# LeCAR-Lab/dial-mpc

Measured on NVIDIA H100. Metric: sample-steps/s (Nsample*Hsample/wall-s) per MPC reverse_once, Go2, higher is better.
Workload: dtype f32

## Files before the change

### dial_mpc_b200/csrc/dial_device.cuh

```cuda
#pragma once

#include <stdint.h>
#include <math.h>
#include "../../include/dial_b200.h"

#ifdef DIAL_HOST_EMUL
#include "warp_emul.h"
#define DEV inline
#define HD inline
inline float __fmaf_rn(float a, float b, float c) { return a * b + c; }
inline float __fadd_rn(float a, float b) { return a + b; }
inline float __fmul_rn(float a, float b) { return a * b; }
inline float __fdiv_rn(float a, float b) { return a / b; }
inline float __fsub_rn(float a, float b) { return a - b; }
inline double __dadd_rn(double a, double b) { return a + b; }
inline double __dsub_rn(double a, double b) { return a - b; }
inline double __dmul_rn(double a, double b) { return a * b; }
inline double __ddiv_rn(double a, double b) { return a / b; }
#else
#define HD __host__ __device__ __forceinline__
#define DEV __device__ __forceinline__
DEV void syncwarp() { __syncwarp(); }
DEV float shfl(float v, int src) { return __shfl_sync(0xffffffffu, v, src); }
DEV float shfl_xor(float v, int m) { return __shfl_xor_sync(0xffffffffu, v, m); }
// ... 8 lines not shown
extern "C" void emul_trace(int kind, int val);
#define DIAL_TRACE(lane, kind, val) do { if ((lane) == 0) emul_trace(kind, val); } while (0)
#else
#define DIAL_TRACE(lane, kind, val) do { } while (0)
#endif

#define DIAL_MAXCHAIN 12
#define DIAL_MAXLEVEL 28
#define DIAL_MAXE 32
#define DIAL_MINVAL 1e-15f
#define DIAL_MINIMP 1e-4f
#define DIAL_MAXIMP 0.9999f

enum { JNT_FREE = 0, JNT_BALL = 1, JNT_SLIDE = 2, JNT_HINGE = 3 };
enum { PAIR_PLANE_SPHERE = 0, PAIR_PLANE_CAPSULE = 1, PAIR_SPHERE_SPHERE = 2, PAIR_SPHERE_CAPSULE = 3, PAIR_CAPSULE_CAPSULE = 4 };

struct alignas(16) DevModel {
  dial_model_desc m;
  int32_t maxdepth;
  int32_t nroot, root_body[4];
  float root_invmass[4];
  int32_t body_rootidx[DIAL_MAXB];
  int32_t body_ndesc[DIAL_MAXB];
  int32_t dof_level[DIAL_MAXV], nlevel;
  int32_t level_adr[DIAL_MAXLEVEL + 1], level_dofs[DIAL_MAXV];
  uint32_t dof_ancmask[DIAL_MAXV];
  uint32_t body_dofmask[DIAL_MAXB];
  int32_t dof_actuator[DIAL_MAXV];
  int32_t dof_limited[DIAL_MAXV];
  int32_t con_pair[DIAL_MAXC], con_sub[DIAL_MAXC];
// ... 7 lines not shown
  int32_t star_nroot, star_nchain, star_maxlen;
  int32_t star_root[8], star_len[4], star_leaf[4], star_att[4];
  int32_t nedge;
  int32_t s_on, s_nrp, s_cs, s_rs, s_npos;
  int32_t s_pos[DIAL_MAXV];
  int32_t s_chain[DIAL_MAXV];
  int32_t s_depth[DIAL_MAXV];
  int32_t s_top[4];
  int32_t s_con_chain[DIAL_MAXC];
  int32_t o_Ms, o_Hs, o_Js, o_xs;
  int32_t sb_on, sb_nroot, sb_root[4], sb_top[4], sb_len[4], sb_att[4];
  int32_t o_xpos, o_xquat, o_xmat, o_xipos, o_cinert, o_cdof, o_cdofdot, o_cvel, o_cacc,
      o_cfrc, o_Mb, o_L, o_J, o_qpos, o_qvel, o_warm, o_ctrl, o_vec, o_frow, o_cpos,
      o_cframe, o_cdist, o_rcom, o_xch, o_crb, o_cfs, o_Md, o_Ld, o_Jd, o_Gd, o_frow2, o_cact, o_hcs, warp_floats;
  int32_t pad_[1];
};

struct alignas(16) DevPlan {
  dial_plan_desc c;
  int32_t pad_[3];
};

#define DIAL_TASK_AT(f) (offsetof(dial_plan_desc, f) - offsetof(dial_plan_desc, vel_cmd) == offsetof(dial_task, f))
static_assert(DIAL_TASK_AT(vel_cmd) && DIAL_TASK_AT(ang_cmd) && DIAL_TASK_AT(pos_tar) && DIAL_TASK_AT(gait_duty) &&
              DIAL_TASK_AT(gait_cadence) && DIAL_TASK_AT(gait_amplitude) && DIAL_TASK_AT(gait_phase) &&
              DIAL_TASK_AT(cmd_step) && DIAL_TASK_AT(cmd_vel) && DIAL_TASK_AT(cmd_ang) && DIAL_TASK_AT(n_stage) &&
              DIAL_TASK_AT(jump_dt) && DIAL_TASK_AT(pose_seq) && DIAL_TASK_AT(yaw_seq) &&
              DIAL_TASK_AT(contact_targets) && DIAL_TASK_AT(contact_radius) && DIAL_TASK_AT(n_user) &&
              DIAL_TASK_AT(user) &&
              offsetof(dial_plan_desc, user) + sizeof(float) * DIAL_MAXUSER - offsetof(dial_plan_desc, vel_cmd) == sizeof(dial_task),
// ... 437 lines not shown
    p = 1.00167406f + p * w; p = 2.83297682f + p * w;
  }
  return p * x;
}
DEV float jax_normal_legacy(uint32_t k0, uint32_t k1, uint32_t i, uint32_t n) {
  uint32_t bits = jax_bits_legacy(k0, k1, i, n);
  float f = __uint_as_float((bits >> 9) | 0x3F800000u) - 1.0f;
  const float lo = -0.99999994f;
  float u = fmaxf(lo, f * 2.0f + lo);
  return 1.41421356237f * erfinv_f32(u);
}

struct WarpCtx {
  const DevModel* M;
  const DevPlan* P;
  float* s;
  int lane;
  int nch;
  int ndesc;
  int mylevel;
  int parent;
  int midsync;
  int itersync;
  float* dbg;
  int chain[DIAL_MAXCHAIN];
  int s_pos;
  int s_col;
  int s_cb;
  int s_chain;
  int s_depth;
// ... 271 lines not shown
  syncwarp();
  float y = 0.f;
  if (w.nch > 0) {
    for (int c = 0; c < M.m.ncon; ++c) {
      const int kc = M.con_lastdof[c];
      if ((M.dof_ancmask[kc] >> lane) & 1u) {
        const int off = M.dof_nchain[kc] - w.nch;
#pragma unroll
        for (int e = 0; e < 4; ++e) y += Jc[(4 * c + e) * MC + off] * frow[4 * c + e];
      }
    }
  }
  return y;
}

DEV void kbi(float timestep, const float* solref, const float* solimp, float pos,
             float& k, float& b, float& imp) {
  float timeconst = fmaxf(solref[0], 2.f * timestep), dampratio = solref[1];
  float dmin = fminf(fmaxf(solimp[0], DIAL_MINIMP), DIAL_MAXIMP);
  float dmax = fminf(fmaxf(solimp[1], DIAL_MINIMP), DIAL_MAXIMP);
  float width = fmaxf(DIAL_MINVAL, solimp[2]);
  float mid = fminf(fmaxf(solimp[3], DIAL_MINIMP), DIAL_MAXIMP);
  float power = fmaxf(1.f, solimp[4]);
  k = 1.f / (dmax * dmax * timeconst * timeconst * dampratio * dampratio);
  b = 2.f / (dmax * timeconst);
  if (solref[0] <= 0.f) k = -solref[0] / (dmax * dmax);
  if (solref[1] <= 0.f) b = -solref[1] / dmax;
  float x = fabsf(pos) / width;
  float y;
  if (power == 2.f) {
    y = x < mid ? x * x / mid : 1.f - (1.f - x) * (1.f - x) / (1.f - mid);
  } else {
    float a_ = (1.f / powf(mid, power - 1.f)) * powf(x, power);
    float b_ = 1.f - (1.f / powf(1.f - mid, power - 1.f)) * powf(fmaxf(1.f - x, 0.f), power);
    y = x < mid ? a_ : b_;
  }
  imp = dmin + y * (dmax - dmin);
  imp = fminf(fmaxf(imp, dmin), dmax);
  if (x > 1.f) imp = dmax;
}

struct Solver {
  float qacc, Ma, grad, search, qfs, qas;
  float l_sign, l_D, l_aref, l_Jaref;
  float e_D, e_aref, e_Jaref;
  float gauss, cost, prev_cost, gradnorm2;
  float qfc;
};

DEV void update_constraint(WarpCtx& w, Solver& S) {
  float fl = (S.l_Jaref < 0.f) ? -S.l_D * S.l_Jaref : 0.f;
  float fe = (S.e_Jaref < 0.f) ? -S.e_D * S.e_Jaref : 0.f;
  float qfc = mul_JT(w, fe) + S.l_sign * fl;
  S.grad = S.Ma - S.qfs - qfc;
// ... 1090 lines not shown
}
DEV V3 frame_tangent(V3 n) {
  V3 alt = (n.y > -0.5f && n.y < 0.5f) ? v3(0, 1, 0) : v3(0, 0, 1);
  float bn;
  return vnormalize(alt - n * dot(n, alt), bn);
}

template <class SH = ShapeRT>
DEV void collide(WarpCtx& w) {
  const DevModel& M = *w.M;
  const dial_model_desc& m = M.m;
  const int lane = w.lane;
  if (lane >= SH::ncon(M)) return;
  const float* xpos = SM(xpos);
  const float* xmat = SM(xmat);
  const int k = M.con_pair[lane];
  const int g1 = m.pair_geom1[k], g2 = m.pair_geom2[k];
  const int b1 = m.geom_bodyid[g1], b2 = m.geom_bodyid[g2];
  const float* X1 = xmat + 9 * b1;
  const float* X2 = xmat + 9 * b2;
  const V3 gp1 = mat_apply(X1, m.geom_pos[g1]) + ld3(xpos + 3 * b1);
  const V3 gp2 = mat_apply(X2, m.geom_pos[g2]) + ld3(xpos + 3 * b2);
  const int kind = SH::pair_kind(M, k);
  V3 n, t1, p;
  float dist;
  if (kind == PAIR_PLANE_SPHERE || kind == PAIR_PLANE_CAPSULE) {
    n = mat_z(X1, m.geom_quat[g1]);
    const float radius = m.geom_size[g2][0];
    V3 center = gp2;
    if (kind == PAIR_PLANE_CAPSULE) {
      V3 ax = mat_z(X2, m.geom_quat[g2]);
      float bn;
      V3 bd = vnormalize(ax - n * dot(n, ax), bn);
// ... 34 lines not shown

template <int NL, int NR, class SH = ShapeRT>
DEV void physics_step(WarpCtx& w, bool integrate) {
  constexpr int MCU = (NL == 3 && NR == 6) ? 9 : DIAL_MAXCHAIN;
  const DevModel& M = *w.M;
  const dial_model_desc& m = M.m;
  const int lane = w.lane, nb = SH::nbody(M), nv = SH::nv(M);
  float* xpos = SM(xpos); float* xquat = SM(xquat); float* xmat = SM(xmat); float* xipos = SM(xipos);
  float* cinert = SM(cinert); float* cdof = SM(cdof); float* cdofdot = SM(cdofdot);
  float* cvel = SM(cvel); float* cacc = SM(cacc); float* cfrc = SM(cfrc);
  float* J = SM(J);
  float* qpos = SM(qpos); float* qvel = SM(qvel); float* warm = SM(warm); float* ctrl = SM(ctrl);
  float* cpos = SM(cpos); float* cframe = SM(cframe); float* cdist = SM(cdist); float* rcom = SM(rcom);

  const int b = lane;
  const bool isbody = b > 0 && b < nb;
  const int depth = isbody ? m.body_depth[b] : -1;
  const int jid = isbody ? m.body_jntadr[b] : -1;
  const int jtype = jid >= 0 ? m.jnt_type[jid] : -1;
  V3 anchor = v3(0, 0, 0), axis = v3(0, 0, 1), xip = v3(0, 0, 0);
  float ximat[9];
#pragma unroll
  for (int i = 0; i < 9; ++i) ximat[i] = 0.f;
  Q4 qL; qL.w = 1.f; qL.x = qL.y = qL.z = 0.f;
  V3 pL = v3(0, 0, 0), aL = v3(0, 0, 0), axL = v3(0, 0, 1);
  if (isbody) {
    const Q4 bq = ldq(m.body_quat[b]);
    const V3 bp = ld3(m.body_pos[b]);
    qL = bq; pL = bp;
    if (jtype == JNT_HINGE || jtype == JNT_SLIDE) {
      const int qa = m.jnt_qposadr[jid];
      const V3 jp = ld3(m.jnt_pos[jid]), ja = ld3(m.jnt_axis[jid]);
      aL = bp + qrot(bq, jp);
      axL = qrot(bq, ja);
      const float dq = qpos[qa] - m.qpos0[qa];
      if (jtype == JNT_HINGE) {
        qL = qmul(bq, axisangle(ja, dq));
        pL = aL - qrot(qL, jp);
      } else {
        pL = bp + axL * dq;
      }
    }
  }
  V3 pos = v3(0, 0, 0);
  Q4 quat; quat.w = 1.f; quat.x = quat.y = quat.z = 0.f;
  for (int lv = 1; lv <= SH::maxdepth(M); ++lv) {
    if (depth == lv) {
      if (jtype == JNT_FREE) {
        const int qa = m.jnt_qposadr[jid];
        pos = ld3(qpos + qa);
        quat = qnormalize(ldq(qpos + qa + 3));
        stq(qpos + qa + 3, quat);
        anchor = pos;
        axis = v3(0, 0, 1);
      } else {
        const int p = m.body_parentid[b];
        const Q4 pq = ldq(xquat + 4 * p);
        const V3 pp = ld3(xpos + 3 * p);
        quat = qmul(pq, qL);
        pos = pp + qrot(pq, pL);
        anchor = pp + qrot(pq, aL);
        axis = qrot(pq, axL);
      }
      quat = qnormalize(quat);
      st3(xpos + 3 * b, pos);
      stq(xquat + 4 * b, quat);
    }
    syncwarp();
  }
  if (isbody) {
    float R[9];
    qmat(quat, R);
#pragma unroll
    for (int i = 0; i < 9; ++i) xmat[9 * b + i] = R[i];
    xip = pos + qrot(quat, ld3(m.body_ipos[b]));
    st3(xipos + 3 * b, xip);
    qmat(qmul(quat, ldq(m.body_iquat[b])), ximat);
  }

  const int myroot = isbody ? M.body_rootidx[b] : -1;
  V3 com = v3(0, 0, 0);
  for (int r = 0; r < SH::nroot(M); ++r) {
    float mass = (myroot == r) ? m.body_mass[b] : 0.f;
    float sx = mass * xip.x, sy = mass * xip.y, sz = mass * xip.z;
    warp_sum3(sx, sy, sz);
    V3 c = v3(sx, sy, sz) * M.root_invmass[r];
    if (lane == 0) st3(rcom + 3 * r, c);
    if (myroot == r) com = c;
  }

  if (isbody) {
    V3 off = xip - com;
    float mass = m.body_mass[b];
    const float* di = m.body_inertia[b];
    float I[6];
    I[0] = ximat[0] * ximat[0] * di[0] + ximat[1] * ximat[1] * di[1] + ximat[2] * ximat[2] * di[2];
    I[1] = ximat[3] * ximat[3] * di[0] + ximat[4] * ximat[4] * di[1] + ximat[5] * ximat[5] * di[2];
    I[2] = ximat[6] * ximat[6] * di[0] + ximat[7] * ximat[7] * di[1] + ximat[8] * ximat[8] * di[2];
    I[3] = ximat[0] * ximat[3] * di[0] + ximat[1] * ximat[4] * di[1] + ximat[2] * ximat[5] * di[2];
    I[4] = ximat[0] * ximat[6] * di[0] + ximat[1] * ximat[7] * di[1] + ximat[2] * ximat[8] * di[2];
    I[5] = ximat[3] * ximat[6] * di[0] + ximat[4] * ximat[7] * di[1] + ximat[5] * ximat[8] * di[2];
    float o2 = dot(off, off);
    float* ci = cinert + CIS * b;
    st4(ci, I[0] + mass * (o2 - off.x * off.x), I[1] + mass * (o2 - off.y * off.y), I[2] + mass * (o2 - off.z * off.z),
        I[3] - mass * off.x * off.y);
    st4(ci + 4, I[4] - mass * off.x * off.z, I[5] - mass * off.y * off.z, mass * off.x, mass * off.y);
    st2(ci + 8, mass * off.z, mass);
    if (jid >= 0) {
      int d = m.jnt_dofadr[jid];
      V3 offset = com - anchor;
      if (jtype == JNT_FREE) {
        for (int i = 0; i < 3; ++i) {
          float* c0 = cdof + CDS * (d + i);
          st4(c0, 0.f, 0.f, 0.f, i == 0 ? 1.f : 0.f);
          st2(c0 + 4, i == 1 ? 1.f : 0.f, i == 2 ? 1.f : 0.f);
          V3 ax = v3(xmat[9 * b + i], xmat[9 * b + 3 + i], xmat[9 * b + 6 + i]);
          V3 cx = cross(ax, offset);
          float* c1 = cdof + CDS * (d + 3 + i);
          st4(c1, ax.x, ax.y, ax.z, cx.x);
          st2(c1 + 4, cx.y, cx.z);
        }
      } else if (jtype == JNT_HINGE) {
        V3 cx = cross(axis, offset);
        st4(cdof + CDS * d, axis.x, axis.y, axis.z, cx.x);
        st2(cdof + CDS * d + 4, cx.y, cx.z);
      } else {
        st4(cdof + CDS * d, 0.f, 0.f, 0.f, axis.x);
        st2(cdof + CDS * d + 4, axis.y, axis.z);
      }
    }
  }
  syncwarp();

  float mycv[6] = {0.f, 0.f, 0.f, 0.f, 0.f, 0.f}, myca[6] = {0.f, 0.f, 0.f, 0.f, 0.f, 0.f};
  for (int lv = 1; lv <= SH::maxdepth(M); ++lv) {
    if (depth == lv) {
      int p = m.body_parentid[b];
      float cv[6], ca[6];
#pragma unroll
      for (int i = 0; i < 6; ++i) { cv[i] = cvel[6 * p + i]; ca[i] = cacc[6 * p + i]; }
      if (jtype == JNT_FREE) {
        int d = m.jnt_dofadr[jid];
        for (int k = 0; k < 3; ++k) {
          float qd = qvel[d + k], cd[6];
          ld6(cdof + CDS * (d + k), cd);
#pragma unroll
          for (int i = 0; i < 6; ++i) cv[i] += cd[i] * qd;
          st4(cdofdot + CDS * (d + k), 0.f, 0.f, 0.f, 0.f);
          st2(cdofdot + CDS * (d + k) + 4, 0.f, 0.f);
        }
        float cvt[6];
#pragma unroll
        for (int i = 0; i < 6; ++i) cvt[i] = cv[i];
        for (int k = 3; k < 6; ++k) {
          float dd[6], cd[6];
          ld6(cdof + CDS * (d + k), cd);
          mcross(cvt, cd, dd);
          float qd = qvel[d + k];
          st6(cdofdot + CDS * (d + k), dd);
#pragma unroll
          for (int i = 0; i < 6; ++i) {
            cv[i] += cd[i] * qd;
            ca[i] += dd[i] * qd;
          }
        }
      } else if (jid >= 0) {
        int d = m.jnt_dofadr[jid];
        float dd[6], cd[6];
        ld6(cdof + CDS * d, cd);
        mcross(cv, cd, dd);
        float qd = qvel[d];
        st6(cdofdot + CDS * d, dd);
#pragma unroll
        for (int i = 0; i < 6; ++i) {
          cv[i] += cd[i] * qd;
          ca[i] += dd[i] * qd;
        }
      }
#pragma unroll
      for (int i = 0; i < 6; ++i) {
        cvel[6 * b + i] = cv[i];
        cacc[6 * b + i] = ca[i];
// ... 66 lines not shown
  float myqvel = isdof ? qvel[d] : 0.f;
  float mycdof[6] = {0.f, 0.f, 0.f, 0.f, 0.f, 0.f};
  constexpr bool STAR = NL > 0;
  constexpr int SNR = STAR ? NR : 1, SNL = STAR ? NL : 1;
  float Mrow[STAR ? 1 : MC], R[STAR ? 1 : MC];
  float Mr[SNR], Mc[SNL], Rr[SNR], Rc[SNL];
#pragma unroll
  for (int a = 0; a < SNR; ++a) { Mr[a] = 0.f; Rr[a] = 0.f; }
#pragma unroll
  for (int q = 0; q < SNL; ++q) { Mc[q] = 0.f; Rc[q] = 0.f; }
  if constexpr (!STAR) {
#pragma unroll
    for (int c = 0; c < MCU; ++c) { Mrow[c] = 0.f; R[c] = 0.f; }
  }
  if (isdof) {
    int bi = m.dof_bodyid[d];
    float f[6];
    {
      float crbb[10];
      ld10(SM(crb) + CIS * bi, crbb);
      ld6(cdof + CDS * d, mycdof);
      inert_mul(crbb, mycdof, f);
    }
    if constexpr (STAR) {
      using SD = StarDims<NL, NR>;
      const float arm = m.dof_armature[d];
      if (w.s_chain >= 0) {
        const int att = M.star_att[w.s_chain];
#pragma unroll
        for (int q = 0; q < NL; ++q)
          if (q <= w.s_depth) { float cd[6]; ld6(cdof + CDS * (w.s_top + q), cd); Mc[q] = dot6(f, cd) + (q == w.s_depth ? arm : 0.f); }
// ... 8 lines not shown
      star_store_row<NL, NR>(SM(Ms) + w.s_pos * SD::RS, Mr, Mc);
    } else {
#pragma unroll
      for (int c = 0; c < MCU; ++c)
        if (c < w.nch) { float cd[6]; ld6(cdof + CDS * w.chain[c], cd); Mrow[c] = dot6(f, cd); }
      Mrow[0] += m.dof_armature[d];
      if constexpr (NL >= 0) {
        float* Mb = SM(Mb);
#pragma unroll
        for (int c = 0; c < MCU; ++c)
          if (c < w.nch) Mb[d * MC + c] = Mrow[c];
      }
    }
    float bias = dot6(mycdof, SM(cfs) + 6 * bi);
    float act = 0.f;
    int a = M.dof_actuator[d];
    if (a >= 0) {
      float c = ctrl[a];
      if (m.actuator_ctrllimited[a]) c = fminf(fmaxf(c, m.actuator_ctrlrange[a][0]), m.actuator_ctrlrange[a][1]);
      float force = m.actuator_gain[a] * c + m.actuator_bias[a][0]
                  + m.actuator_bias[a][1] * qpos[m.actuator_qposadr[a]] + m.actuator_bias[a][2] * myqvel;
      if (m.actuator_forcelimited[a]) force = fminf(fmaxf(force, m.actuator_forcerange[a][0]), m.actuator_forcerange[a][1]);
      act = force * m.actuator_gear[a];
    }
    S.qfs = -m.dof_damping[d] * myqvel - bias + act;
  }
  if constexpr (NL >= 0) {
    if (M.s_on && M.o_crb == M.o_Hs) {
      syncwarp();
      float* z = SM(crb);
      for (int i = lane; i < (CIS + 6) * nb; i += 32) z[i] = 0.f;
// ... 13 lines not shown
      for (int a = 0; a < NR; ++a)
        if (a < w.s_depth) { Mr[a] = Ms[a * SD::RS + w.s_depth]; Ms[w.s_pos * SD::RS + a] = Mr[a]; }
    }
  }

  float qacc, qacc_int;
  if constexpr (NL < 0) {
    if (w.midsync) cta_sync();
    else syncwarp();
    qacc = dense_constraint_solve<NR>(w, S, Mrow, myqvel, qacc_int);
  } else if constexpr (STAR) {
  using SD = StarDims<NL, NR>;
  float* Js = SM(Js);
  if (isdof) {
    V3 ca_ = v3(mycdof[0], mycdof[1], mycdof[2]), cl_ = v3(mycdof[3], mycdof[4], mycdof[5]);
    V3 rc = ld3(rcom + 3 * M.body_rootidx[m.dof_bodyid[d]]);
    for (int c = 0; c < SH::ncon(M); ++c) {
      if (!((w.s_conmask >> c) & 1u)) continue;
      const int k = M.con_pair[c];
      float e0 = 0.f, e1 = 0.f, e2 = 0.f, e3 = 0.f;
      const bool moves = (M.body_dofmask[m.geom_bodyid[m.pair_geom2[k]]] >> d) & 1u;
      if (moves && cdist[c] - (m.pair_margin[k] - m.pair_gap[k]) < 0.f) {
        V3 p = ld3(cpos + 3 * c);
        V3 jp = cl_ + cross(ca_, p - rc);
        float jn = dot(ld3(cframe + 9 * c), jp), j1 = dot(ld3(cframe + 9 * c + 3), jp), j2 = dot(ld3(cframe + 9 * c + 6), jp);
        float mu0 = m.pair_friction[k][0], mu1 = m.pair_friction[k][1];
        e0 = jn + mu0 * j1; e1 = jn - mu0 * j1; e2 = jn + mu1 * j2; e3 = jn - mu1 * j2;
      }
      float* col = Js + 4 * c * SD::RS + w.s_col;
      col[0] = e0; col[SD::RS] = e1; col[2 * SD::RS] = e2; col[3 * SD::RS] = e3;
    }
    int lj = M.dof_limited[d];
    if (lj >= 0) {
      float qv = qpos[m.jnt_qposadr[lj]];
      float dmin = qv - m.jnt_range[lj][0], dmax = m.jnt_range[lj][1] - qv;
      float pos = fminf(dmin, dmax) - m.jnt_margin[lj];
      if (pos < 0.f) {
        float sign = dmin < dmax ? 1.f : -1.f;
        float k_, b_, imp;
        kbi(m.timestep, m.jnt_solref[lj], m.jnt_solimp[lj], pos, k_, b_, imp);
        float Rr_ = fmaxf(m.dof_invweight0[d] * (1.f - imp) / imp, DIAL_MINVAL);
        S.l_sign = sign;
        S.l_D = 1.f / Rr_;
        S.l_aref = -b_ * (sign * myqvel) - k_ * imp * pos;
      }
    }
  }
  float ejv, dummy;
  star_mul_MJ<NL, NR, false, true, SH>(w, Mr, Mc, myqvel, dummy, ejv);
  if (lane < SH::nedge(M)) {
    int c = lane >> 2;
    int k = M.con_pair[c];
    float pos = cdist[c] - (m.pair_margin[k] - m.pair_gap[k]);
    if (pos < 0.f) {
      int b1 = m.geom_bodyid[m.pair_geom1[k]], b2 = m.geom_bodyid[m.pair_geom2[k]];
      float mu = m.pair_friction[k][0];
      float t = m.body_invweight0[b1] + m.body_invweight0[b2];
      float iw = (t + mu * mu * t) * 2.f * mu * mu / m.impratio;
      float k_, b_, imp;
      kbi(m.timestep, m.pair_solref[k], m.pair_solimp[k], pos, k_, b_, imp);
      float Rr_ = fmaxf(iw * (1.f - imp) / imp, DIAL_MINVAL);
      S.e_D = 1.f / Rr_;
      S.e_aref = -b_ * ejv - k_ * imp * pos;
    }
  }
  if (w.midsync) cta_sync();
  const float scale = m.meaninertia * (float)(nv > 1 ? nv : 1);
  const float mywarm = isdof ? warm[d] : 0.f;
  float g = S.qfs;
#pragma unroll
  for (int a = 0; a < NR; ++a) Rr[a] = Mr[a];
#pragma unroll
  for (int q = 0; q < NL; ++q) Rc[q] = Mc[q];
  int it = 0;
  bool done;
// ... 36 lines not shown
    float mv, e_jv;
    star_mul_MJ<NL, NR, true, true, SH>(w, Mr, Mc, S.search, mv, e_jv);
    linesearch_core<SH>(w, S, mv, e_jv);
    ++it;
    star_update_constraint<NL, NR, SH>(w, S);
    done = it >= SH::iterations(M);
    float improvement = (S.prev_cost - S.cost) / scale;
    float gradient = sqrtf(S.gradnorm2) / scale;
    if (SH::iterations(M) != 1) done = done || (improvement < m.tolerance) || (gradient < m.tolerance);
  }
  qacc = S.qacc;
  qacc_int = qacc;
  } else {
  if (isdof) {
    V3 ca_ = v3(mycdof[0], mycdof[1], mycdof[2]), cl_ = v3(mycdof[3], mycdof[4], mycdof[5]);
    int rootb = M.body_rootidx[m.dof_bodyid[d]];
    V3 rc = ld3(rcom + 3 * rootb);
    for (int c = 0; c < m.ncon; ++c) {
      const int kc = M.con_lastdof[c];
      if (!((M.dof_ancmask[kc] >> d) & 1u)) continue;
      const int k = M.con_pair[c];
      const int p_ = M.dof_nchain[kc] - w.nch;
      float e0 = 0.f, e1 = 0.f, e2 = 0.f, e3 = 0.f;
      if (cdist[c] - (m.pair_margin[k] - m.pair_gap[k]) < 0.f) {
        V3 p = ld3(cpos + 3 * c);
        V3 jp = cl_ + cross(ca_, p - rc);
        float jn = dot(ld3(cframe + 9 * c), jp), j1 = dot(ld3(cframe + 9 * c + 3), jp), j2 = dot(ld3(cframe + 9 * c + 6), jp);
        float mu0 = m.pair_friction[k][0], mu1 = m.pair_friction[k][1];
        e0 = jn + mu0 * j1; e1 = jn - mu0 * j1; e2 = jn + mu1 * j2; e3 = jn - mu1 * j2;
      }
      J[(4 * c + 0) * MC + p_] = e0; J[(4 * c + 1) * MC + p_] = e1;
      J[(4 * c + 2) * MC + p_] = e2; J[(4 * c + 3) * MC + p_] = e3;
    }
    int lj = M.dof_limited[d];
    if (lj >= 0) {
      float qv = qpos[m.jnt_qposadr[lj]];
      float dmin = qv - m.jnt_range[lj][0], dmax = m.jnt_range[lj][1] - qv;
      float pos = fminf(dmin, dmax) - m.jnt_margin[lj];
      if (pos < 0.f) {
        float sign = dmin < dmax ? 1.f : -1.f;
        float k_, b_, imp;
        kbi(m.timestep, m.jnt_solref[lj], m.jnt_solimp[lj], pos, k_, b_, imp);
        float Rr = fmaxf(m.dof_invweight0[d] * (1.f - imp) / imp, DIAL_MINVAL);
        S.l_sign = sign;
        S.l_D = 1.f / Rr;
        S.l_aref = -b_ * (sign * myqvel) - k_ * imp * pos;
      }
    }
  }
  float ejv = mul_J(w, myqvel);
  if (lane < M.nedge) {
    int c = lane >> 2;
    int k = M.con_pair[c];
    float pos = cdist[c] - (m.pair_margin[k] - m.pair_gap[k]);
    if (pos < 0.f) {
      int b1 = m.geom_bodyid[m.pair_geom1[k]], b2 = m.geom_bodyid[m.pair_geom2[k]];
      float mu = m.pair_friction[k][0];
      float t = m.body_invweight0[b1] + m.body_invweight0[b2];
      float iw = (t + mu * mu * t) * 2.f * mu * mu / m.impratio;
      float k_, b_, imp;
      kbi(m.timestep, m.pair_solref[k], m.pair_solimp[k], pos, k_, b_, imp);
      float Rr = fmaxf(iw * (1.f - imp) / imp, DIAL_MINVAL);
      S.e_D = 1.f / Rr;
      S.e_aref = -b_ * ejv - k_ * imp * pos;
    }
  }

  if (w.midsync) cta_sync();
  const float scale = m.meaninertia * (float)(nv > 1 ? nv : 1);
  const float mywarm = isdof ? warm[d] : 0.f;
  float g = S.qfs;
#pragma unroll
  for (int c = 0; c < MCU; ++c) R[c] = Mrow[c];
  int phase = 0, it = 0;
  while (true) {
    float x = tree_solve<NL, NR, MCU>(w, R, g);
// ... 33 lines not shown
    phase = 1;
    build_H<MCU>(w, S, Mrow, R);
    g = S.grad;
  }
  qacc = S.qacc;
  qacc_int = qacc;

  }

  syncwarp();
  if (isdof) {
    warm[d] = qacc;
    if (integrate) qvel[d] = myqvel + m.timestep * qacc_int;
  }
  syncwarp();
  if (integrate && isbody && jid >= 0) {
    int qa = m.jnt_qposadr[jid], dd = m.jnt_dofadr[jid];
    if (jtype == JNT_FREE) {
      for (int i = 0; i < 3; ++i) qpos[qa + i] += m.timestep * qvel[dd + i];
      V3 wv = ld3(qvel + dd + 3);
      float nrm = sqrtf(dot(wv, wv));
      V3 ax = wv * (1.f / (nrm + 1e-6f * (nrm == 0.f ? 1.f : 0.f)));
      Q4 qn = qnormalize(qmul(ldq(qpos + qa + 3), axisangle(ax, m.timestep * nrm)));
      stq(qpos + qa + 3, qn);
    } else {
      qpos[qa] += m.timestep * qvel[dd];
    }
  }
  syncwarp();
}

DEV float foot_step(float duty, float cadence, float amplitude, float phase, float time) {
// ... 153 lines not shown
    float r_pos = -dot(dp, dp);
    float dy = quat_yaw(bk.rot) - T.yaw_seq[stage];
    float r_yaw = -dy * dy;
    const float r_contact = part0, pen = part1;
    rew = r_pos + r_upright + 0.3f * r_yaw + 0.1f * r_contact - 0.1f * pen + 10.f;
    int ns = (int)floorf((float)(step + 1) * c.dt / T.jump_dt);
    stage = ns < T.n_stage - 1 ? ns : T.n_stage - 1;
  }
  return rew;
}

template <int NL, int NR, class SH = ShapeRT>
DEV void rollout_warp(const DevModel* Mp, const DevPlan* Pp, float* slab, const RolloutArgs& A,
                      int row, int lane) {
  WarpCtx w;
  w.M = Mp; w.P = Pp; w.s = slab; w.lane = lane;
  w.midsync = A.lockstep >= 2;
  w.itersync = A.lockstep >= 3;
  w.dbg = A.dbg;
  const DevModel& M = *Mp;
  const dial_model_desc& m = M.m;
  const dial_plan_desc& c = Pp->c;
  const int nq = SH::nq(M), nv = SH::nv(M), nu = SH::nu(M), nb = SH::nbody(M);
  const int inst = A.rows_per_inst > 0 ? row / A.rows_per_inst : 0;
  const int lrow = row - inst * A.rows_per_inst;
  w.nch = 0; w.ndesc = 0; w.mylevel = -1; w.parent = -1;
#pragma unroll
  for (int i = 0; i < DIAL_MAXCHAIN; ++i) w.chain[i] = 0;
  if (lane < nv) {
    w.nch = M.dof_nchain[lane];
    w.ndesc = M.dof_ndesc[lane];
// ... 137 lines not shown
```

### dial_mpc_b200/csrc/dial_host.h

```cpp
#pragma once
#include <string.h>
#include <string>
#include "dial_device.cuh"

#ifndef DIAL_MAXTHREADS
#define DIAL_MAXTHREADS 512
#endif
#ifndef DIAL_DENSE_NV
#define DIAL_DENSE_NV 22
#endif
static_assert(DIAL_DENSE_NV >= 1 && DIAL_DENSE_NV <= 32, "the dense solver keeps one matrix row per lane");

static inline void derive_star(const dial_model_desc& m, DevModel& D) {
  const int nv = m.nv;
  D.star_nroot = D.star_nchain = D.star_maxlen = 0;
  int nchild[DIAL_MAXV] = {0};
  for (int i = 0; i < nv; ++i) if (m.dof_parentid[i] >= 0) nchild[m.dof_parentid[i]]++;
  bool inchain[DIAL_MAXV] = {false};
  int nchain = 0, len[4], leaf[4], top[4];
  for (int i = 0; i < nv; ++i) {
    if (nchild[i] != 0) continue;
    int l = 0, j = i, t = i;
    while (j >= 0 && nchild[j] <= 1) { inchain[j] = true; t = j; ++l; j = m.dof_parentid[j]; }
    if (nchain >= 4) return;
// ... 226 lines not shown
  } else { D.o_Mb = D.o_L = D.o_J = D.o_xch = 0; }
  D.o_qpos = take(m.nq); D.o_qvel = take(nv); D.o_warm = take(nv); D.o_ctrl = take(m.nu);
  D.o_vec = take(32); D.o_frow = take(32); D.o_cpos = take(3 * m.ncon); D.o_cframe = take(9 * m.ncon);
  D.o_cdist = take(m.ncon); D.o_rcom = take(3 * 4);
  const int ncrb = (CIS + 6) * nb;
  const bool crb_in_Hs = !D.dense && D.s_on && ncrb <= D.s_npos * D.s_rs;
  const bool crb_in_Md = D.dense && ncrb <= nv * nv;
  if (!crb_in_Hs && !crb_in_Md) { D.o_crb = take(CIS * nb); D.o_cfs = take(6 * nb); }
  if (D.dense) {
    D.o_Md = take(nv * nv); D.o_Ld = 0; D.o_Jd = take(D.nrow_c * D.jd_stride); D.o_Gd = take(6 * nv);
    D.o_frow2 = take(D.nrow_c); D.o_cact = take(DIAL_MAXC); D.o_hcs = D.o_vec;
  }
  if (crb_in_Hs) { D.o_crb = D.o_Hs; D.o_cfs = D.o_Hs + CIS * nb; }
  if (crb_in_Md) { D.o_crb = D.o_Md; D.o_cfs = D.o_Md + CIS * nb; }
  D.warp_floats = o;
  return true;
}

static inline const char* instance_model_difference(const DevModel& plan, const DevModel& inst) {
  const dial_model_desc &a = plan.m, &b = inst.m;
#define DIAL_SAME(f) if (memcmp(&a.f, &b.f, sizeof(a.f)) != 0) return #f;
  DIAL_SAME(nq) DIAL_SAME(nv) DIAL_SAME(nu) DIAL_SAME(nbody) DIAL_SAME(njnt) DIAL_SAME(ngeom) DIAL_SAME(nsite)
  DIAL_SAME(ncon) DIAL_SAME(npair) DIAL_SAME(iterations) DIAL_SAME(ls_iterations) DIAL_SAME(eulerdamp) DIAL_SAME(cone)
  DIAL_SAME(timestep)
  DIAL_SAME(body_parentid) DIAL_SAME(body_rootid) DIAL_SAME(body_depth) DIAL_SAME(body_jntadr) DIAL_SAME(body_dofadr)
  DIAL_SAME(body_dofnum) DIAL_SAME(jnt_type) DIAL_SAME(jnt_qposadr) DIAL_SAME(jnt_dofadr) DIAL_SAME(jnt_limited)
  DIAL_SAME(jnt_range) DIAL_SAME(dof_bodyid) DIAL_SAME(dof_jntid) DIAL_SAME(dof_parentid) DIAL_SAME(geom_type)
  DIAL_SAME(geom_bodyid) DIAL_SAME(pair_kind) DIAL_SAME(pair_geom1) DIAL_SAME(pair_geom2) DIAL_SAME(pair_ncon)
  DIAL_SAME(pair_condim) DIAL_SAME(site_bodyid) DIAL_SAME(actuator_dofadr) DIAL_SAME(actuator_qposadr)
  DIAL_SAME(actuator_ctrllimited) DIAL_SAME(actuator_forcelimited) DIAL_SAME(actuator_ctrlrange)
#undef DIAL_SAME
  const size_t off = offsetof(DevModel, maxdepth), inv = offsetof(DevModel, root_invmass);
  const char *pa = reinterpret_cast<const char*>(&plan), *pb = reinterpret_cast<const char*>(&inst);
  if (memcmp(pa + off, pb + off, inv - off) != 0 ||
      memcmp(pa + inv + sizeof(plan.root_invmass), pb + inv + sizeof(plan.root_invmass),
             sizeof(DevModel) - inv - sizeof(plan.root_invmass)) != 0)
    return "derived structure";
  return nullptr;
}

static inline bool task_valid(const dial_task& t) {
  return t.n_stage >= 1 && t.n_stage <= DIAL_MAXSTAGE && t.n_user >= 0 && t.n_user <= DIAL_MAXUSER;
}

static inline int star_variant(const DevModel& D) {
  if (D.dense) return D.m.nv == DIAL_DENSE_NV ? 3 : -1;
  if (D.star_nchain >= 1 && D.star_nchain <= 4) {
    int maxchain = 0;
    for (int i = 0; i < D.m.nv; ++i) maxchain = D.dof_nchain[i] > maxchain ? D.dof_nchain[i] : maxchain;
    if (D.star_nroot == 6 && D.star_maxlen <= 3 && maxchain <= 9) return 1;
    if (D.star_nroot == 7 && D.star_maxlen <= 5) return 2;
// ... 5 lines not shown
```

### dial_mpc_b200/csrc/dial_rollout_variant.cu

```cuda
#include <cuda_runtime.h>
#include "dial_host.h"

#ifndef DIAL_VARIANT
#error "compile with -DDIAL_VARIANT=<0..4>"
#endif
#if DIAL_VARIANT == 1
#define DIAL_V_NL 3
#define DIAL_V_NR 6
#elif DIAL_VARIANT == 2
#define DIAL_V_NL 5
#define DIAL_V_NR 7
#elif DIAL_VARIANT == 3
#define DIAL_V_NL -1
#define DIAL_V_NR DIAL_DENSE_NV
#elif DIAL_VARIANT == 4
#define DIAL_V_NL 5
#define DIAL_V_NR 6
#else
#define DIAL_V_NL 0
#define DIAL_V_NR 0
#endif

__device__ __forceinline__ uint32_t smem_u32(const void* p) { return (uint32_t)__cvta_generic_to_shared(p); }
__device__ __forceinline__ void mbar_init(uint64_t* bar, int count) {
// ... 4 lines not shown
  asm volatile("mbarrier.arrive.expect_tx.shared::cta.b64 _, [%0], %1;" ::"r"(smem_u32(bar)), "r"(bytes) : "memory");
}
__device__ __forceinline__ void tma_bulk_g2s(void* dst, const void* src, uint32_t bytes, uint64_t* bar) {
  asm volatile("cp.async.bulk.shared::cluster.global.mbarrier::complete_tx::bytes [%0], [%1], %2, [%3];"
               ::"r"(smem_u32(dst)), "l"(src), "r"(bytes), "r"(smem_u32(bar)) : "memory");
}
__device__ __forceinline__ void mbar_wait(uint64_t* bar, uint32_t parity) {
  asm volatile(
      "{\n .reg .pred p;\n WAIT_%=:\n"
      " mbarrier.try_wait.parity.shared::cta.b64 p, [%0], %1;\n"
      " @p bra DONE_%=;\n bra WAIT_%=;\n DONE_%=:\n}\n" ::"r"(smem_u32(bar)), "r"(parity) : "memory");
}

static_assert(sizeof(DevModel) % 16 == 0, "DevModel must be a multiple of 16 bytes for cp.async.bulk");
static_assert(sizeof(DevPlan) % 16 == 0, "DevPlan must be a multiple of 16 bytes for cp.async.bulk");

template <int NL, int NR, class SH = ShapeRT>
__global__ void __launch_bounds__(DIAL_MAXTHREADS, 1) rollout_kernel(const DevModel* __restrict__ gM,
                                                         const DevPlan* __restrict__ gP,
                                                         const RolloutArgs A) {
  extern __shared__ __align__(128) unsigned char smem[];
  __shared__ __align__(8) uint64_t bar;
  DevModel* sM = reinterpret_cast<DevModel*>(smem);
  DevPlan* sP = reinterpret_cast<DevPlan*>(smem + sizeof(DevModel));
  float* slabs = reinterpret_cast<float*>(smem + sizeof(DevModel) + sizeof(DevPlan));
  const int warp = threadIdx.x >> 5, lane = threadIdx.x & 31, wpc = blockDim.x >> 5;
  if (threadIdx.x == 0) {
    if (A.models) gM = A.models + (model_rows(A) > 0 ? blockIdx.x / ((model_rows(A) + wpc - 1) / wpc) : 0);
    mbar_init(&bar, 1);
    mbar_expect_tx(&bar, (uint32_t)(sizeof(DevModel) + sizeof(DevPlan)));
    tma_bulk_g2s(sM, gM, (uint32_t)sizeof(DevModel), &bar);
    tma_bulk_g2s(sP, gP, (uint32_t)sizeof(DevPlan), &bar);
  }
  __syncthreads();
  mbar_wait(&bar, 0);
  float* slab = slabs + (size_t)warp * sM->warp_floats;
  if constexpr (NL < 0) {
    if (A.row_counter) {
      for (;;) {
        int row = 0;
        if (lane == 0) row = (int)atomicAdd(A.row_counter, 1u);
        row = __shfl_sync(0xffffffffu, row, 0);
        if (row >= A.nrows) return;
        rollout_warp<NL, NR>(sM, sP, slab, A, row, lane);
        __syncwarp();
      }
    }
  }
  int row = blockIdx.x * wpc + warp;
  bool active = true;
// ... 62 lines not shown
```

Measured before the change: 76.15 million.

## Precompute per-lane model index table in shared memory to cut indirect lookups

Adds a 64-byte-per-lane LaneRec table to DevModel, built by warp 0 after the model is staged into shared memory. It caches body, joint, dof and contact indices, the local joint anchor and axis, and the per-edge contact constants (stiffness, damping, inverse weight, margin). Kinematics, contact, Jacobian and constraint code read these precomputed fields instead of chaining indirect loads and recomputing kbi coefficients every step. The cost is a one-time table build per CTA plus an extra __syncthreads, and indices are narrowed to int8.

```diff
diff --git a/dial_mpc_b200/csrc/dial_device.cuh b/dial_mpc_b200/csrc/dial_device.cuh
--- a/dial_mpc_b200/csrc/dial_device.cuh
+++ b/dial_mpc_b200/csrc/dial_device.cuh
@@ -46,6 +46,18 @@
 
 enum { JNT_FREE = 0, JNT_BALL = 1, JNT_SLIDE = 2, JNT_HINGE = 3 };
 enum { PAIR_PLANE_SPHERE = 0, PAIR_PLANE_CAPSULE = 1, PAIR_SPHERE_SPHERE = 2, PAIR_SPHERE_CAPSULE = 3, PAIR_CAPSULE_CAPSULE = 4 };
+
+struct alignas(16) LaneRec {
+  int8_t depth, jid, jtype, qa, da, par, root, dbody, act, lj, ljqa, droot, cb1, cb2, cg1, cg2;
+  uint32_t cmask;
+  int8_t ek, pad_[3];
+  float aL[3], axL[3];
+  float ek_, eb_, eiw, emg;
+};
+static_assert(sizeof(LaneRec) == 64, "LaneRec: 64 bytes per lane (2 KB per CTA)");
+static_assert(DIAL_MAXQ <= 127 && DIAL_MAXV <= 127 && DIAL_MAXB <= 127 && DIAL_MAXG <= 127 && DIAL_MAXP <= 127 &&
+              DIAL_MAXU <= 127, "LaneRec keeps indices in int8_t");
+struct alignas(16) LaneTab { LaneRec r[32]; };
 
 struct alignas(16) DevModel {
   dial_model_desc m;
@@ -83,6 +95,7 @@
       o_cfrc, o_Mb, o_L, o_J, o_qpos, o_qvel, o_warm, o_ctrl, o_vec, o_frow, o_cpos,
       o_cframe, o_cdist, o_rcom, o_xch, o_crb, o_cfs, o_Md, o_Ld, o_Jd, o_Gd, o_frow2, o_cact, o_hcs, warp_floats;
   int32_t pad_[1];
+  LaneTab lt;
 };
 
 struct alignas(16) DevPlan {
@@ -550,6 +563,7 @@
 struct WarpCtx {
   const DevModel* M;
   const DevPlan* P;
+  const LaneRec* L;
   float* s;
   int lane;
   int nch;
@@ -851,18 +865,21 @@
   return y;
 }
 
-DEV void kbi(float timestep, const float* solref, const float* solimp, float pos,
-             float& k, float& b, float& imp) {
+DEV void kbi_coef(float timestep, const float* solref, const float* solimp, float& k, float& b) {
   float timeconst = fmaxf(solref[0], 2.f * timestep), dampratio = solref[1];
+  float dmax = fminf(fmaxf(solimp[1], DIAL_MINIMP), DIAL_MAXIMP);
+  k = 1.f / (dmax * dmax * timeconst * timeconst * dampratio * dampratio);
+  b = 2.f / (dmax * timeconst);
+  if (solref[0] <= 0.f) k = -solref[0] / (dmax * dmax);
+  if (solref[1] <= 0.f) b = -solref[1] / dmax;
+}
+
+DEV void kbi_imp(const float* solimp, float pos, float& imp) {
   float dmin = fminf(fmaxf(solimp[0], DIAL_MINIMP), DIAL_MAXIMP);
   float dmax = fminf(fmaxf(solimp[1], DIAL_MINIMP), DIAL_MAXIMP);
   float width = fmaxf(DIAL_MINVAL, solimp[2]);
   float mid = fminf(fmaxf(solimp[3], DIAL_MINIMP), DIAL_MAXIMP);
   float power = fmaxf(1.f, solimp[4]);
-  k = 1.f / (dmax * dmax * timeconst * timeconst * dampratio * dampratio);
-  b = 2.f / (dmax * timeconst);
-  if (solref[0] <= 0.f) k = -solref[0] / (dmax * dmax);
-  if (solref[1] <= 0.f) b = -solref[1] / dmax;
   float x = fabsf(pos) / width;
   float y;
   if (power == 2.f) {
@@ -875,6 +892,65 @@
   imp = dmin + y * (dmax - dmin);
   imp = fminf(fmaxf(imp, dmin), dmax);
   if (x > 1.f) imp = dmax;
+}
+
+DEV void kbi(float timestep, const float* solref, const float* solimp, float pos,
+             float& k, float& b, float& imp) {
+  kbi_coef(timestep, solref, solimp, k, b);
+  kbi_imp(solimp, pos, imp);
+}
+
+DEV void lane_table_build(const DevModel& M, LaneTab* T, int lane) {
+  const dial_model_desc& m = M.m;
+  const int i = lane;
+  LaneRec r;
+  const bool isbody = i > 0 && i < m.nbody;
+  const int jid = isbody ? m.body_jntadr[i] : -1;
+  const int jtype = jid >= 0 ? m.jnt_type[jid] : -1;
+  r.depth = (int8_t)(isbody ? m.body_depth[i] : -1);
+  r.jid = (int8_t)jid;
+  r.jtype = (int8_t)jtype;
+  r.qa = (int8_t)(jid >= 0 ? m.jnt_qposadr[jid] : 0);
+  r.da = (int8_t)(jid >= 0 ? m.jnt_dofadr[jid] : 0);
+  r.par = (int8_t)(isbody ? m.body_parentid[i] : 0);
+  r.root = (int8_t)(isbody ? M.body_rootidx[i] : -1);
+  r.aL[0] = r.aL[1] = r.aL[2] = 0.f;
+  r.axL[0] = r.axL[1] = 0.f; r.axL[2] = 1.f;
+  if (jtype == JNT_HINGE || jtype == JNT_SLIDE) {
+    const Q4 bq = ldq(m.body_quat[i]);
+    const V3 bp = ld3(m.body_pos[i]);
+    st3(r.aL, bp + qrot(bq, ld3(m.jnt_pos[jid])));
+    st3(r.axL, qrot(bq, ld3(m.jnt_axis[jid])));
+  }
+  const bool isdof = i < m.nv;
+  const int dbody = isdof ? m.dof_bodyid[i] : 0;
+  const int lj = isdof ? M.dof_limited[i] : -1;
+  r.dbody = (int8_t)dbody;
+  r.act = (int8_t)(isdof ? M.dof_actuator[i] : -1);
+  r.lj = (int8_t)lj;
+  r.ljqa = (int8_t)(lj >= 0 ? m.jnt_qposadr[lj] : 0);
+  r.droot = (int8_t)(isdof ? M.body_rootidx[dbody] : 0);
+  r.cg1 = r.cg2 = r.cb1 = r.cb2 = 0; r.cmask = 0u;
+  if (i < m.ncon) {
+    const int k = M.con_pair[i];
+    const int g1 = m.pair_geom1[k], g2 = m.pair_geom2[k];
+    r.cg1 = (int8_t)g1; r.cg2 = (int8_t)g2;
+    r.cb1 = (int8_t)m.geom_bodyid[g1]; r.cb2 = (int8_t)m.geom_bodyid[g2];
+    r.cmask = M.body_dofmask[m.geom_bodyid[g2]];
+  }
+  r.ek = 0; r.ek_ = r.eb_ = r.eiw = r.emg = 0.f;
+  if (i < M.nedge) {
+    const int k = M.con_pair[i >> 2];
+    r.ek = (int8_t)k;
+    r.emg = m.pair_margin[k] - m.pair_gap[k];
+    const int b1 = m.geom_bodyid[m.pair_geom1[k]], b2 = m.geom_bodyid[m.pair_geom2[k]];
+    const float mu = m.pair_friction[k][0];
+    const float t = m.body_invweight0[b1] + m.body_invweight0[b2];
+    r.eiw = (t + mu * mu * t) * 2.f * mu * mu / m.impratio;
+    kbi_coef(m.timestep, m.pair_solref[k], m.pair_solimp[k], r.ek_, r.eb_);
+  }
+  r.pad_[0] = r.pad_[1] = r.pad_[2] = 0;
+  T->r[i] = r;
 }
 
 struct Solver {
@@ -1995,9 +2071,10 @@
   if (lane >= SH::ncon(M)) return;
   const float* xpos = SM(xpos);
   const float* xmat = SM(xmat);
+  const LaneRec& LC = w.L[lane];
   const int k = M.con_pair[lane];
-  const int g1 = m.pair_geom1[k], g2 = m.pair_geom2[k];
-  const int b1 = m.geom_bodyid[g1], b2 = m.geom_bodyid[g2];
+  const int g1 = LC.cg1, g2 = LC.cg2;
+  const int b1 = LC.cb1, b2 = LC.cb2;
   const float* X1 = xmat + 9 * b1;
   const float* X2 = xmat + 9 * b2;
   const V3 gp1 = mat_apply(X1, m.geom_pos[g1]) + ld3(xpos + 3 * b1);
@@ -2062,10 +2139,10 @@
   float* cpos = SM(cpos); float* cframe = SM(cframe); float* cdist = SM(cdist); float* rcom = SM(rcom);
 
   const int b = lane;
+  const LaneRec& LR = w.L[lane];
   const bool isbody = b > 0 && b < nb;
-  const int depth = isbody ? m.body_depth[b] : -1;
-  const int jid = isbody ? m.body_jntadr[b] : -1;
-  const int jtype = jid >= 0 ? m.jnt_type[jid] : -1;
+  const int depth = LR.depth;
+  const int jtype = LR.jtype;
   V3 anchor = v3(0, 0, 0), axis = v3(0, 0, 1), xip = v3(0, 0, 0);
   float ximat[9];
 #pragma unroll
@@ -2077,14 +2154,14 @@
     const V3 bp = ld3(m.body_pos[b]);
     qL = bq; pL = bp;
     if (jtype == JNT_HINGE || jtype == JNT_SLIDE) {
-      const int qa = m.jnt_qposadr[jid];
-      const V3 jp = ld3(m.jnt_pos[jid]), ja = ld3(m.jnt_axis[jid]);
-      aL = bp + qrot(bq, jp);
-      axL = qrot(bq, ja);
+      aL = ld3(LR.aL);
+      axL = ld3(LR.axL);
+      const int qa = LR.qa;
       const float dq = qpos[qa] - m.qpos0[qa];
       if (jtype == JNT_HINGE) {
-        qL = qmul(bq, axisangle(ja, dq));
-        pL = aL - qrot(qL, jp);
+        const int jid = LR.jid;
+        qL = qmul(bq, axisangle(ld3(m.jnt_axis[jid]), dq));
+        pL = aL - qrot(qL, ld3(m.jnt_pos[jid]));
       } else {
         pL = bp + axL * dq;
       }
@@ -2095,14 +2172,14 @@
   for (int lv = 1; lv <= SH::maxdepth(M); ++lv) {
     if (depth == lv) {
       if (jtype == JNT_FREE) {
-        const int qa = m.jnt_qposadr[jid];
+        const int qa = LR.qa;
         pos = ld3(qpos + qa);
         quat = qnormalize(ldq(qpos + qa + 3));
         stq(qpos + qa + 3, quat);
         anchor = pos;
         axis = v3(0, 0, 1);
       } else {
-        const int p = m.body_parentid[b];
+        const int p = LR.par;
         const Q4 pq = ldq(xquat + 4 * p);
         const V3 pp = ld3(xpos + 3 * p);
         quat = qmul(pq, qL);
@@ -2126,7 +2203,7 @@
     qmat(qmul(quat, ldq(m.body_iquat[b])), ximat);
   }
 
-  const int myroot = isbody ? M.body_rootidx[b] : -1;
+  const int myroot = LR.root;
   V3 com = v3(0, 0, 0);
   for (int r = 0; r < SH::nroot(M); ++r) {
     float mass = (myroot == r) ? m.body_mass[b] : 0.f;
@@ -2154,8 +2231,8 @@
         I[3] - mass * off.x * off.y);
     st4(ci + 4, I[4] - mass * off.x * off.z, I[5] - mass * off.y * off.z, mass * off.x, mass * off.y);
     st2(ci + 8, mass * off.z, mass);
-    if (jid >= 0) {
-      int d = m.jnt_dofadr[jid];
+    if (jtype >= 0) {
+      int d = LR.da;
       V3 offset = com - anchor;
       if (jtype == JNT_FREE) {
         for (int i = 0; i < 3; ++i) {
@@ -2183,12 +2260,12 @@
   float mycv[6] = {0.f, 0.f, 0.f, 0.f, 0.f, 0.f}, myca[6] = {0.f, 0.f, 0.f, 0.f, 0.f, 0.f};
   for (int lv = 1; lv <= SH::maxdepth(M); ++lv) {
     if (depth == lv) {
-      int p = m.body_parentid[b];
+      int p = LR.par;
       float cv[6], ca[6];
 #pragma unroll
       for (int i = 0; i < 6; ++i) { cv[i] = cvel[6 * p + i]; ca[i] = cacc[6 * p + i]; }
       if (jtype == JNT_FREE) {
-        int d = m.jnt_dofadr[jid];
+        int d = LR.da;
         for (int k = 0; k < 3; ++k) {
           float qd = qvel[d + k], cd[6];
           ld6(cdof + CDS * (d + k), cd);
@@ -2212,8 +2289,8 @@
             ca[i] += dd[i] * qd;
           }
         }
-      } else if (jid >= 0) {
-        int d = m.jnt_dofadr[jid];
+      } else if (jtype >= 0) {
+        int d = LR.da;
         float dd[6], cd[6];
         ld6(cdof + CDS * d, cd);
         mcross(cv, cd, dd);
@@ -2310,7 +2387,7 @@
     for (int c = 0; c < MCU; ++c) { Mrow[c] = 0.f; R[c] = 0.f; }
   }
   if (isdof) {
-    int bi = m.dof_bodyid[d];
+    int bi = LR.dbody;
     float f[6];
     {
       float crbb[10];
@@ -2349,7 +2426,7 @@
     }
     float bias = dot6(mycdof, SM(cfs) + 6 * bi);
     float act = 0.f;
-    int a = M.dof_actuator[d];
+    int a = LR.act;
     if (a >= 0) {
       float c = ctrl[a];
       if (m.actuator_ctrllimited[a]) c = fminf(fmaxf(c, m.actuator_ctrlrange[a][0]), m.actuator_ctrlrange[a][1]);
@@ -2393,25 +2470,25 @@
   float* Js = SM(Js);
   if (isdof) {
     V3 ca_ = v3(mycdof[0], mycdof[1], mycdof[2]), cl_ = v3(mycdof[3], mycdof[4], mycdof[5]);
-    V3 rc = ld3(rcom + 3 * M.body_rootidx[m.dof_bodyid[d]]);
+    V3 rc = ld3(rcom + 3 * LR.droot);
     for (int c = 0; c < SH::ncon(M); ++c) {
       if (!((w.s_conmask >> c) & 1u)) continue;
-      const int k = M.con_pair[c];
+      const LaneRec& LE = w.L[4 * c];
       float e0 = 0.f, e1 = 0.f, e2 = 0.f, e3 = 0.f;
-      const bool moves = (M.body_dofmask[m.geom_bodyid[m.pair_geom2[k]]] >> d) & 1u;
-      if (moves && cdist[c] - (m.pair_margin[k] - m.pair_gap[k]) < 0.f) {
+      const bool moves = (w.L[c].cmask >> d) & 1u;
+      if (moves && cdist[c] - LE.emg < 0.f) {
         V3 p = ld3(cpos + 3 * c);
         V3 jp = cl_ + cross(ca_, p - rc);
         float jn = dot(ld3(cframe + 9 * c), jp), j1 = dot(ld3(cframe + 9 * c + 3), jp), j2 = dot(ld3(cframe + 9 * c + 6), jp);
-        float mu0 = m.pair_friction[k][0], mu1 = m.pair_friction[k][1];
+        float mu0 = m.pair_friction[LE.ek][0], mu1 = m.pair_friction[LE.ek][1];
         e0 = jn + mu0 * j1; e1 = jn - mu0 * j1; e2 = jn + mu1 * j2; e3 = jn - mu1 * j2;
       }
       float* col = Js + 4 * c * SD::RS + w.s_col;
       col[0] = e0; col[SD::RS] = e1; col[2 * SD::RS] = e2; col[3 * SD::RS] = e3;
     }
-    int lj = M.dof_limited[d];
+    int lj = LR.lj;
     if (lj >= 0) {
-      float qv = qpos[m.jnt_qposadr[lj]];
+      float qv = qpos[LR.ljqa];
       float dmin = qv - m.jnt_range[lj][0], dmax = m.jnt_range[lj][1] - qv;
       float pos = fminf(dmin, dmax) - m.jnt_margin[lj];
       if (pos < 0.f) {
@@ -2429,15 +2506,11 @@
   star_mul_MJ<NL, NR, false, true, SH>(w, Mr, Mc, myqvel, dummy, ejv);
   if (lane < SH::nedge(M)) {
     int c = lane >> 2;
-    int k = M.con_pair[c];
-    float pos = cdist[c] - (m.pair_margin[k] - m.pair_gap[k]);
+    float pos = cdist[c] - LR.emg;
     if (pos < 0.f) {
-      int b1 = m.geom_bodyid[m.pair_geom1[k]], b2 = m.geom_bodyid[m.pair_geom2[k]];
-      float mu = m.pair_friction[k][0];
-      float t = m.body_invweight0[b1] + m.body_invweight0[b2];
-      float iw = (t + mu * mu * t) * 2.f * mu * mu / m.impratio;
-      float k_, b_, imp;
-      kbi(m.timestep, m.pair_solref[k], m.pair_solimp[k], pos, k_, b_, imp);
+      const float iw = LR.eiw, k_ = LR.ek_, b_ = LR.eb_;
+      float imp;
+      kbi_imp(m.pair_solimp[LR.ek], pos, imp);
       float Rr_ = fmaxf(iw * (1.f - imp) / imp, DIAL_MINVAL);
       S.e_D = 1.f / Rr_;
       S.e_aref = -b_ * ejv - k_ * imp * pos;
@@ -2504,27 +2577,26 @@
   } else {
   if (isdof) {
     V3 ca_ = v3(mycdof[0], mycdof[1], mycdof[2]), cl_ = v3(mycdof[3], mycdof[4], mycdof[5]);
-    int rootb = M.body_rootidx[m.dof_bodyid[d]];
-    V3 rc = ld3(rcom + 3 * rootb);
+    V3 rc = ld3(rcom + 3 * LR.droot);
     for (int c = 0; c < m.ncon; ++c) {
       const int kc = M.con_lastdof[c];
       if (!((M.dof_ancmask[kc] >> d) & 1u)) continue;
-      const int k = M.con_pair[c];
+      const LaneRec& LE = w.L[4 * c];
       const int p_ = M.dof_nchain[kc] - w.nch;
       float e0 = 0.f, e1 = 0.f, e2 = 0.f, e3 = 0.f;
-      if (cdist[c] - (m.pair_margin[k] - m.pair_gap[k]) < 0.f) {
+      if (cdist[c] - LE.emg < 0.f) {
         V3 p = ld3(cpos + 3 * c);
         V3 jp = cl_ + cross(ca_, p - rc);
         float jn = dot(ld3(cframe + 9 * c), jp), j1 = dot(ld3(cframe + 9 * c + 3), jp), j2 = dot(ld3(cframe + 9 * c + 6), jp);
-        float mu0 = m.pair_friction[k][0], mu1 = m.pair_friction[k][1];
+        float mu0 = m.pair_friction[LE.ek][0], mu1 = m.pair_friction[LE.ek][1];
         e0 = jn + mu0 * j1; e1 = jn - mu0 * j1; e2 = jn + mu1 * j2; e3 = jn - mu1 * j2;
       }
       J[(4 * c + 0) * MC + p_] = e0; J[(4 * c + 1) * MC + p_] = e1;
       J[(4 * c + 2) * MC + p_] = e2; J[(4 * c + 3) * MC + p_] = e3;
     }
-    int lj = M.dof_limited[d];
+    int lj = LR.lj;
     if (lj >= 0) {
-      float qv = qpos[m.jnt_qposadr[lj]];
+      float qv = qpos[LR.ljqa];
       float dmin = qv - m.jnt_range[lj][0], dmax = m.jnt_range[lj][1] - qv;
       float pos = fminf(dmin, dmax) - m.jnt_margin[lj];
       if (pos < 0.f) {
@@ -2541,15 +2613,11 @@
   float ejv = mul_J(w, myqvel);
   if (lane < M.nedge) {
     int c = lane >> 2;
-    int k = M.con_pair[c];
-    float pos = cdist[c] - (m.pair_margin[k] - m.pair_gap[k]);
+    float pos = cdist[c] - LR.emg;
     if (pos < 0.f) {
-      int b1 = m.geom_bodyid[m.pair_geom1[k]], b2 = m.geom_bodyid[m.pair_geom2[k]];
-      float mu = m.pair_friction[k][0];
-      float t = m.body_invweight0[b1] + m.body_invweight0[b2];
-      float iw = (t + mu * mu * t) * 2.f * mu * mu / m.impratio;
-      float k_, b_, imp;
-      kbi(m.timestep, m.pair_solref[k], m.pair_solimp[k], pos, k_, b_, imp);
+      const float iw = LR.eiw, k_ = LR.ek_, b_ = LR.eb_;
+      float imp;
+      kbi_imp(m.pair_solimp[LR.ek], pos, imp);
       float Rr = fmaxf(iw * (1.f - imp) / imp, DIAL_MINVAL);
       S.e_D = 1.f / Rr;
       S.e_aref = -b_ * ejv - k_ * imp * pos;
@@ -2613,8 +2681,8 @@
     if (integrate) qvel[d] = myqvel + m.timestep * qacc_int;
   }
   syncwarp();
-  if (integrate && isbody && jid >= 0) {
-    int qa = m.jnt_qposadr[jid], dd = m.jnt_dofadr[jid];
+  if (integrate && isbody && jtype >= 0) {
+    int qa = LR.qa, dd = LR.da;
     if (jtype == JNT_FREE) {
       for (int i = 0; i < 3; ++i) qpos[qa + i] += m.timestep * qvel[dd + i];
       V3 wv = ld3(qvel + dd + 3);
@@ -2798,7 +2866,7 @@
 DEV void rollout_warp(const DevModel* Mp, const DevPlan* Pp, float* slab, const RolloutArgs& A,
                       int row, int lane) {
   WarpCtx w;
-  w.M = Mp; w.P = Pp; w.s = slab; w.lane = lane;
+  w.M = Mp; w.P = Pp; w.L = Mp->lt.r; w.s = slab; w.lane = lane;
   w.midsync = A.lockstep >= 2;
   w.itersync = A.lockstep >= 3;
   w.dbg = A.dbg;
diff --git a/dial_mpc_b200/csrc/dial_host.h b/dial_mpc_b200/csrc/dial_host.h
--- a/dial_mpc_b200/csrc/dial_host.h
+++ b/dial_mpc_b200/csrc/dial_host.h
@@ -264,6 +264,9 @@
   if (crb_in_Hs) { D.o_crb = D.o_Hs; D.o_cfs = D.o_Hs + CIS * nb; }
   if (crb_in_Md) { D.o_crb = D.o_Md; D.o_cfs = D.o_Md + CIS * nb; }
   D.warp_floats = o;
+#ifdef DIAL_HOST_EMUL
+  for (int lane = 0; lane < 32; ++lane) lane_table_build(D, &D.lt, lane);
+#endif
   return true;
 }
 
@@ -284,7 +287,7 @@
   const char *pa = reinterpret_cast<const char*>(&plan), *pb = reinterpret_cast<const char*>(&inst);
   if (memcmp(pa + off, pb + off, inv - off) != 0 ||
       memcmp(pa + inv + sizeof(plan.root_invmass), pb + inv + sizeof(plan.root_invmass),
-             sizeof(DevModel) - inv - sizeof(plan.root_invmass)) != 0)
+             offsetof(DevModel, lt) - inv - sizeof(plan.root_invmass)) != 0)
     return "derived structure";
   return nullptr;
 }
diff --git a/dial_mpc_b200/csrc/dial_rollout_variant.cu b/dial_mpc_b200/csrc/dial_rollout_variant.cu
--- a/dial_mpc_b200/csrc/dial_rollout_variant.cu
+++ b/dial_mpc_b200/csrc/dial_rollout_variant.cu
@@ -42,6 +42,8 @@
 
 static_assert(sizeof(DevModel) % 16 == 0, "DevModel must be a multiple of 16 bytes for cp.async.bulk");
 static_assert(sizeof(DevPlan) % 16 == 0, "DevPlan must be a multiple of 16 bytes for cp.async.bulk");
+constexpr size_t kStagedModel = offsetof(DevModel, lt);
+static_assert(kStagedModel % 16 == 0, "the staged part of DevModel must be a multiple of 16 bytes for cp.async.bulk");
 
 template <int NL, int NR, class SH = ShapeRT>
 __global__ void __launch_bounds__(DIAL_MAXTHREADS, 1) rollout_kernel(const DevModel* __restrict__ gM,
@@ -56,12 +58,14 @@
   if (threadIdx.x == 0) {
     if (A.models) gM = A.models + (model_rows(A) > 0 ? blockIdx.x / ((model_rows(A) + wpc - 1) / wpc) : 0);
     mbar_init(&bar, 1);
-    mbar_expect_tx(&bar, (uint32_t)(sizeof(DevModel) + sizeof(DevPlan)));
-    tma_bulk_g2s(sM, gM, (uint32_t)sizeof(DevModel), &bar);
+    mbar_expect_tx(&bar, (uint32_t)(kStagedModel + sizeof(DevPlan)));
+    tma_bulk_g2s(sM, gM, (uint32_t)kStagedModel, &bar);
     tma_bulk_g2s(sP, gP, (uint32_t)sizeof(DevPlan), &bar);
   }
   __syncthreads();
   mbar_wait(&bar, 0);
+  if (warp == 0) lane_table_build(*sM, &sM->lt, lane);
+  __syncthreads();
   float* slab = slabs + (size_t)warp * sM->warp_floats;
   if constexpr (NL < 0) {
     if (A.row_counter) {
```

After: 75.34 million, median of 6. -1.1%, worse.
